# DLR-RM/AugmentedAutoencoder

Hardware: NVIDIA H100
Metric: pose queries/sec (encode+codebook NN) (higher is better)
Workload: dtype f32 via split-fp16 tensor-core products (3x, fp32 accumulate)

## Files before the change

augmentedautoencoder_b200/csrc/tc_common.cuh:

```cuda
#pragma once
#include <cuda.h>
#include <cuda_fp16.h>
#include <cuda_runtime.h>
#include <stdint.h>

namespace aae {
namespace tc {

__device__ __forceinline__ uint32_t smem_u32(const void* p) { return (uint32_t)__cvta_generic_to_shared(p); }

__device__ __forceinline__ bool elect_one() {
  uint32_t pred = 0;
  asm volatile(
      "{\n\t"
      ".reg .pred P1;\n\t"
      "elect.sync _|P1, 0xffffffff;\n\t"
      "selp.b32 %0, 1, 0, P1;\n\t"
      "}\n"
      : "=r"(pred));
  return pred != 0;
}

__device__ __forceinline__ void mbar_init(uint64_t* bar, uint32_t count) {
  asm volatile("mbarrier.init.shared::cta.b64 [%0], %1;" ::"r"(smem_u32(bar)), "r"(count));
}
__device__ __forceinline__ void fence_barrier_init() { asm volatile("fence.mbarrier_init.release.cluster;" ::: "memory"); }
__device__ __forceinline__ void fence_proxy_async_smem() { asm volatile("fence.proxy.async.shared::cta;" ::: "memory"); }

__device__ __forceinline__ void mbar_arrive_expect_tx(uint64_t* bar, uint32_t bytes) {
  asm volatile("mbarrier.arrive.expect_tx.shared::cta.b64 _, [%0], %1;" ::"r"(smem_u32(bar)), "r"(bytes) : "memory");
}
__device__ __forceinline__ void mbar_arrive(uint64_t* bar) {
  asm volatile("mbarrier.arrive.shared::cta.b64 _, [%0];" ::"r"(smem_u32(bar)) : "memory");
}
__device__ __forceinline__ bool mbar_try_wait(uint64_t* bar, uint32_t parity) {
  uint32_t ok;
  asm volatile(
      "{\n\t"
      ".reg .pred P1;\n\t"
      "mbarrier.try_wait.parity.shared::cta.b64 P1, [%1], %2;\n\t"
      "selp.b32 %0, 1, 0, P1;\n\t"
      "}\n"
      : "=r"(ok)
      : "r"(smem_u32(bar)), "r"(parity)
      : "memory");
  return ok != 0;
}
__device__ __forceinline__ void mbar_wait(uint64_t* bar, uint32_t parity) {
  while (!mbar_try_wait(bar, parity)) {
  }
}

__device__ __forceinline__ void prefetch_tmap(const CUtensorMap* m) {
  asm volatile("prefetch.tensormap [%0];" ::"l"(reinterpret_cast<uint64_t>(m)) : "memory");
}
__device__ __forceinline__ void tma_load_2d(void* smem_dst, const CUtensorMap* m, uint64_t* bar, int c0, int c1) {
  asm volatile("cp.async.bulk.tensor.2d.shared::cluster.global.mbarrier::complete_tx::bytes [%0], [%1, {%3, %4}], [%2];" ::"r"(
                   smem_u32(smem_dst)),
               "l"(reinterpret_cast<uint64_t>(m)), "r"(smem_u32(bar)), "r"(c0), "r"(c1)
               : "memory");
}
__device__ __forceinline__ void tma_load_4d(void* smem_dst, const CUtensorMap* m, uint64_t* bar, int c0, int c1, int c2, int c3) {
  asm volatile(
      "cp.async.bulk.tensor.4d.shared::cluster.global.mbarrier::complete_tx::bytes [%0], [%1, {%3, %4, %5, %6}], [%2];" ::"r"(
          smem_u32(smem_dst)),
      "l"(reinterpret_cast<uint64_t>(m)), "r"(smem_u32(bar)), "r"(c0), "r"(c1), "r"(c2), "r"(c3)
      : "memory");
}

__device__ __forceinline__ void bulk_store_1d(void* gmem_dst, const void* smem_src, uint32_t bytes) {
  asm volatile("cp.async.bulk.global.shared::cta.bulk_group [%0], [%1], %2;" ::"l"(gmem_dst), "r"(smem_u32(smem_src)), "r"(bytes) : "memory");
}
__device__ __forceinline__ void bulk_commit_group() { asm volatile("cp.async.bulk.commit_group;" ::: "memory"); }
__device__ __forceinline__ void bulk_wait_read_all() { asm volatile("cp.async.bulk.wait_group.read 0;" ::: "memory"); }
__device__ __forceinline__ void bulk_wait_all() { asm volatile("cp.async.bulk.wait_group 0;" ::: "memory"); }
__device__ __forceinline__ void tma_store_2d(const CUtensorMap* m, const void* smem_src, int c0, int c1) {
  asm volatile("cp.async.bulk.tensor.2d.global.shared::cta.bulk_group [%0, {%2, %3}], [%1];" ::"l"(reinterpret_cast<uint64_t>(m)),
               "r"(smem_u32(smem_src)), "r"(c0), "r"(c1)
               : "memory");
}
__device__ __forceinline__ void tma_store_5d(const CUtensorMap* m, const void* smem_src, int c0, int c1, int c2, int c3, int c4) {
  asm volatile("cp.async.bulk.tensor.5d.global.shared::cta.bulk_group [%0, {%2, %3, %4, %5, %6}], [%1];" ::"l"(reinterpret_cast<uint64_t>(m)),
               "r"(smem_u32(smem_src)), "r"(c0), "r"(c1), "r"(c2), "r"(c3), "r"(c4)
               : "memory");
}

template <int N>
struct Wgmma;
#define AAE_D8(i) "+f"(d[i]), "+f"(d[i + 1]), "+f"(d[i + 2]), "+f"(d[i + 3]), "+f"(d[i + 4]), "+f"(d[i + 5]), "+f"(d[i + 6]), "+f"(d[i + 7])
template <>
struct Wgmma<64> {
  template <int TA, int TB>
  static __device__ __forceinline__ void ss(float (&d)[32], uint64_t da, uint64_t db, uint32_t accumulate) {
    asm volatile(
        "{\n\t.reg .pred p;\n\tsetp.ne.b32 p, %34, 0;\n\t"
        "wgmma.mma_async.sync.aligned.m64n64k16.f32.f16.f16 {%0, %1, %2, %3, %4, %5, %6, %7, %8, %9, %10, %11, %12, %13, %14, %15, %16, %17, %18, %19, %20, %21, %22, %23, %24, %25, %26, %27, %28, %29, %30, %31}, %32, %33, p, 1, 1, %35, %36;\n\t}\n"
        : AAE_D8(0), AAE_D8(8), AAE_D8(16), AAE_D8(24)
        : "l"(da), "l"(db), "r"(accumulate), "n"(TA), "n"(TB));
  }
};

template <>
struct Wgmma<128> {
  template <int TA, int TB>
  static __device__ __forceinline__ void ss(float (&d)[64], uint64_t da, uint64_t db, uint32_t accumulate) {
    asm volatile(
        "{\n\t.reg .pred p;\n\tsetp.ne.b32 p, %66, 0;\n\t"
        "wgmma.mma_async.sync.aligned.m64n128k16.f32.f16.f16 {%0, %1, %2, %3, %4, %5, %6, %7, %8, %9, %10, %11, %12, %13, %14, %15, %16, %17, %18, %19, %20, %21, %22, %23, %24, %25, %26, %27, %28, %29, %30, %31, %32, %33, %34, %35, %36, %37, %38, %39, %40, %41, %42, %43, %44, %45, %46, %47, %48, %49, %50, %51, %52, %53, %54, %55, %56, %57, %58, %59, %60, %61, %62, %63}, %64, %65, p, 1, 1, %67, %68;\n\t}\n"
        : AAE_D8(0), AAE_D8(8), AAE_D8(16), AAE_D8(24), AAE_D8(32), AAE_D8(40), AAE_D8(48), AAE_D8(56)
        : "l"(da), "l"(db), "r"(accumulate), "n"(TA), "n"(TB));
  }
};

__device__ __forceinline__ void wgmma_fence() { asm volatile("wgmma.fence.sync.aligned;" ::: "memory"); }
__device__ __forceinline__ void wgmma_commit() { asm volatile("wgmma.commit_group.sync.aligned;" ::: "memory"); }
template <int N>
__device__ __forceinline__ void wgmma_wait() { asm volatile("wgmma.wait_group.sync.aligned %0;" ::"n"(N) : "memory"); }
template <int R>
__device__ __forceinline__ void wgmma_fence_regs(float (&d)[R]) {
#pragma unroll
  for (int i = 0; i < R; ++i) asm volatile("" : "+f"(d[i])::"memory");
}

template <int N>
__device__ __forceinline__ void setmaxnreg_dec() { asm volatile("setmaxnreg.dec.sync.aligned.u32 %0;" ::"n"(N)); }
template <int N>
__device__ __forceinline__ void setmaxnreg_inc() { asm volatile("setmaxnreg.inc.sync.aligned.u32 %0;" ::"n"(N)); }

__device__ __forceinline__ void cp_async_16(void* smem_dst, const void* gmem_src, bool pred) {
  const int bytes = pred ? 16 : 0;
  asm volatile("cp.async.cg.shared.global [%0], [%1], 16, %2;" ::"r"(smem_u32(smem_dst)), "l"(gmem_src), "r"(bytes) : "memory");
}
__device__ __forceinline__ void cp_async_wait_all() { asm volatile("cp.async.wait_all;" ::: "memory"); }
__device__ __forceinline__ void named_bar_sync(int id, int threads) { asm volatile("bar.sync %0, %1;" ::"r"(id), "r"(threads) : "memory"); }

__device__ __forceinline__ uint64_t make_sw128_kmajor_desc(uint32_t smem_addr) {
  uint64_t d = 0;
  d |= (uint64_t)((smem_addr & 0x3FFFF) >> 4);
  d |= (uint64_t)1 << 16;
  d |= (uint64_t)(1024 >> 4) << 32;
  d |= (uint64_t)1 << 62;
  return d;
}
__device__ __forceinline__ uint64_t make_sw128_mnmajor_desc(uint32_t smem_addr, uint32_t lbo_bytes, uint32_t sbo_bytes) {
  uint64_t d = 0;
  d |= (uint64_t)((smem_addr & 0x3FFFF) >> 4);
  d |= (uint64_t)(lbo_bytes >> 4) << 16;
  d |= (uint64_t)(sbo_bytes >> 4) << 32;
  d |= (uint64_t)1 << 62;
  return d;
}
__device__ __forceinline__ uint64_t desc_advance_k(uint64_t desc, int k_step) { return desc + (uint64_t)((k_step * 32) >> 4); }

__device__ __forceinline__ void split_f16(float x, __half& hi, __half& lo) {
  hi = __float2half_rn(x);
  lo = __float2half_rn(x - __half2float(hi));
}

__device__ __forceinline__ void split_f16x2(float a, float b, uint32_t& hi2, uint32_t& lo2) {
  const float ca = __fmul_rn(a, 8193.0f), cb = __fmul_rn(b, 8193.0f);
  const float ha = __fsub_rn(ca, __fsub_rn(ca, a)), hb = __fsub_rn(cb, __fsub_rn(cb, b));
  const __half2 h = __floats2half2_rn(ha, hb);
  const __half2 l = __floats2half2_rn(__fsub_rn(a, ha), __fsub_rn(b, hb));
  hi2 = *reinterpret_cast<const uint32_t*>(&h);
  lo2 = *reinterpret_cast<const uint32_t*>(&l);
}

}

typedef CUresult (*PFN_tmapEncodeTiled)(CUtensorMap*, CUtensorMapDataType, cuuint32_t, void*, const cuuint64_t*, const cuuint64_t*,
                                        const cuuint32_t*, const cuuint32_t*, CUtensorMapInterleave, CUtensorMapSwizzle,
                                        CUtensorMapL2promotion, CUtensorMapFloatOOBfill);
PFN_tmapEncodeTiled get_tmap_encoder();
int make_tmap_f16(CUtensorMap* out, const void* base, int rank, const uint64_t* dims, const uint64_t* strides_bytes, const uint32_t* box,
                  int swizzle_bytes = 128);

}
```

augmentedautoencoder_b200/csrc/tc_gemm.cu:

```cuda
#include <limits.h>

#include <algorithm>
#include <vector>

#include "tc.cuh"
#include "tc_common.cuh"
#include "tc_plan.cuh"

namespace aae {

using namespace tc;

PFN_tmapEncodeTiled get_tmap_encoder() {
  static PFN_tmapEncodeTiled fn = nullptr;
  if (!fn) {
    void* p = nullptr;
    cudaDriverEntryPointQueryResult q;
    if (cudaGetDriverEntryPoint("cuTensorMapEncodeTiled", &p, cudaEnableDefault, &q) == cudaSuccess && q == cudaDriverEntryPointSuccess)
      fn = reinterpret_cast<PFN_tmapEncodeTiled>(p);
  }
  return fn;
}

int make_tmap_f16(CUtensorMap* out, const void* base, int rank, const uint64_t* dims, const uint64_t* strides_bytes, const uint32_t* box,
                  int swizzle_bytes) {
  PFN_tmapEncodeTiled enc = get_tmap_encoder();
  if (!enc) { set_error("cuTensorMapEncodeTiled is unavailable in this driver"); return AAE_ERR_CUDA; }
  cuuint64_t gdim[5], gstr[4];
  cuuint32_t bx[5], es[5];
  for (int i = 0; i < rank; ++i) { gdim[i] = dims[i]; bx[i] = box[i]; es[i] = 1; }
  for (int i = 0; i + 1 < rank; ++i) gstr[i] = strides_bytes[i];
  CUresult r = enc(out, CU_TENSOR_MAP_DATA_TYPE_FLOAT16, (cuuint32_t)rank, const_cast<void*>(base), gdim, gstr, bx, es,
                   CU_TENSOR_MAP_INTERLEAVE_NONE, swizzle_bytes == 64 ? CU_TENSOR_MAP_SWIZZLE_64B : CU_TENSOR_MAP_SWIZZLE_128B,
                   CU_TENSOR_MAP_L2_PROMOTION_L2_256B,
                   CU_TENSOR_MAP_FLOAT_OOB_FILL_NONE);
  if (r != CUDA_SUCCESS) { set_error("cuTensorMapEncodeTiled failed with CUresult %d (rank %d)", (int)r, rank); return AAE_ERR_CUDA; }
  return AAE_OK;
}

template <int N_TILE, int W_STAGES, int PLANES = 2>
struct TcSmem {
  static constexpr int W_BYTES = N_TILE * TC_KCH * 2;
  static constexpr int W_STAGE_BYTES = PLANES * W_BYTES;
  static constexpr int BODY = TC_A_RING_BYTES + W_STAGES * W_STAGE_BYTES;
  static constexpr int TOTAL = BODY + 1024  + 256 ;
};

struct TcTile {
  int m0, n0, z, u_begin, u_end;
};
template <int N_TILE>
__device__ __forceinline__ TcTile tc_tile(const TcGemmParams& p, const TcTiles& g, int t) {
  TcTile r;
  const int yz = t / g.n;
  const int y = yz % g.m;
  r.z = yz / g.m;
  r.m0 = y * 128;
  r.n0 = (t - yz * g.n) * N_TILE;
  r.u_begin = r.z * p.units_per_split;
  r.u_end = min(p.groups * p.chunks_per_tap, r.u_begin + p.units_per_split);
  return r;
}

template <int N_TILE, int W_STAGES, int PLANES = 2>
__global__ void __launch_bounds__(TC_THREADS, 1)
tc_gemm_kernel(const __grid_constant__ CUtensorMap tm_a_hi, const __grid_constant__ CUtensorMap tm_a_lo,
               const __grid_constant__ CUtensorMap tm_w_hi, const __grid_constant__ CUtensorMap tm_w_lo, const TcGemmParams p,
               const TcTiles tiles) {
  using S = TcSmem<N_TILE, W_STAGES, PLANES>;
  constexpr int R = N_TILE / 2;
  extern __shared__ uint8_t smem_raw[];
  uint8_t* smem = reinterpret_cast<uint8_t*>((reinterpret_cast<uintptr_t>(smem_raw) + 1023) & ~(uintptr_t)1023);
  uint64_t* a_full = reinterpret_cast<uint64_t*>(smem + S::BODY);
  uint64_t* a_empty = a_full + TC_A_SLOTS_MAX;
  uint64_t* w_full = a_empty + TC_A_SLOTS_MAX;
  uint64_t* w_empty = w_full + W_STAGES;
  uint8_t* w_ring = smem + TC_A_RING_BYTES;
  const int a_plane = p.a_rows * TC_KCH * 2, a_slot = PLANES * a_plane;

  const int warp = threadIdx.x >> 5;
  const int lane = threadIdx.x & 31;

  if (threadIdx.x == 0) {
    prefetch_tmap(&tm_a_hi);
    if constexpr (PLANES == 2) prefetch_tmap(&tm_a_lo);
    prefetch_tmap(&tm_w_hi);
    if constexpr (PLANES == 2) prefetch_tmap(&tm_w_lo);
    for (int s = 0; s < p.a_slots; ++s) { mbar_init(&a_full[s], 1); mbar_init(&a_empty[s], 2); }
    for (int s = 0; s < W_STAGES; ++s) { mbar_init(&w_full[s], 1); mbar_init(&w_empty[s], 2); }
    fence_barrier_init();
  }
  __syncthreads();

  if (warp < 4) {
    setmaxnreg_dec<TC_PRODUCER_REGS>();
    if (warp == 0 && lane == 0) {
      const int hw = p.OH * p.OW;
      int ia = 0, iw = 0;
      for (int t = blockIdx.x; t < tiles.count; t += gridDim.x) {
        const TcTile T = tc_tile<N_TILE>(p, tiles, t);
        const int b0 = T.m0 / hw, rem = T.m0 - b0 * hw;
        const int oh0 = rem / p.OW, ow0 = rem - oh0 * p.OW;
        for (int u = T.u_begin; u < T.u_end; ++u, ++ia) {
          const int g = u / p.chunks_per_tap, cc = u - g * p.chunks_per_tap;
          const int sa = ia & (p.a_slots - 1);
          mbar_wait(&a_empty[sa], (ia & p.a_slots) ? 0u : 1u);
          uint8_t* a = smem + sa * a_slot;
          mbar_arrive_expect_tx(&a_full[sa], a_slot);
          const int c0 = p.grp_ch[g] + cc * TC_KCH;
          const int x = ow0 + p.grp_dx[g], y = oh0 + p.grp_dy[g];
          tma_load_4d(a, &tm_a_hi, &a_full[sa], c0, x, y, b0);
          if constexpr (PLANES == 2) tma_load_4d(a + a_plane, &tm_a_lo, &a_full[sa], c0, x, y, b0);
          const int first = p.grp_first[g], ntaps = p.grp_ntaps[g];
          for (int k = 0; k < ntaps; ++k, ++iw) {
            const int sw = iw % W_STAGES;
            mbar_wait(&w_empty[sw], ((uint32_t)(iw / W_STAGES) & 1u) ^ 1u);
            uint8_t* w = w_ring + sw * S::W_STAGE_BYTES;
            mbar_arrive_expect_tx(&w_full[sw], S::W_STAGE_BYTES);
            const int kcol = (p.grp_tap[first + k] * p.chunks_per_tap + cc) * TC_KCH;
            tma_load_2d(w, &tm_w_hi, &w_full[sw], kcol, T.n0);
            if constexpr (PLANES == 2) tma_load_2d(w + S::W_BYTES, &tm_w_lo, &w_full[sw], kcol, T.n0);
          }
        }
      }
    }
  } else {
    setmaxnreg_inc<TC_CONSUMER_REGS>();
    const int wg = (warp - 4) >> 2;
    const bool releases = (warp & 3) == 0 && lane == 0;
    constexpr int H = R / 8;
    float acc[R], crs[R], v[R];
#pragma unroll
    for (int j = 0; j < R; ++j) { acc[j] = 0.f; crs[j] = 0.f; v[j] = 0.f; }
    int pt = 0, half = 2;
    auto epilogue_half = [&](int h) {
      const TcTile P = tc_tile<N_TILE>(p, tiles, pt);
      if (h == 0) tc_epilogue_frag<PLANES, 0, H>(p, v, P.m0 + wg * 64, P.n0, P.z, warp, lane);
      else tc_epilogue_frag<PLANES, H, 2 * H>(p, v, P.m0 + wg * 64, P.n0, P.z, warp, lane);
    };
    int ia = 0, iw = 0;
    for (int t = blockIdx.x; t < tiles.count; t += gridDim.x) {
      const TcTile T = tc_tile<N_TILE>(p, tiles, t);
      for (int u = T.u_begin; u < T.u_end; ++u, ++ia) {
        const int g = u / p.chunks_per_tap;
        const int sa = ia & (p.a_slots - 1);
        mbar_wait(&a_full[sa], (ia & p.a_slots) ? 1u : 0u);
        const int first = p.grp_first[g], ntaps = p.grp_ntaps[g];
        for (int k = 0; k < ntaps; ++k, ++iw) {
          const int sw = iw % W_STAGES;
          mbar_wait(&w_full[sw], (uint32_t)(iw / W_STAGES) & 1u);
          const uint32_t a_tap = smem_u32(smem + sa * a_slot) + (uint32_t)((wg * p.a_wg_rows + p.grp_row[first + k]) * TC_KCH * 2);
          const uint32_t st = smem_u32(w_ring + sw * S::W_STAGE_BYTES);
          const uint64_t a_hi = make_sw128_kmajor_desc(a_tap);
          const uint64_t a_lo = make_sw128_kmajor_desc(a_tap + (uint32_t)a_plane);
          const uint64_t w_hi = make_sw128_kmajor_desc(st);
          const uint64_t w_lo = make_sw128_kmajor_desc(st + S::W_BYTES);
          const bool accumulate = u > T.u_begin || k > 0;
          wgmma_fence_regs(acc);
          if constexpr (PLANES == 2) wgmma_fence_regs(crs);
          wgmma_fence();
#pragma unroll
          for (int kk = 0; kk < TC_KCH / 16; ++kk) {
            const uint32_t scale_d = (accumulate || kk > 0) ? 1u : 0u;
            Wgmma<N_TILE>::template ss<0, 0>(acc, desc_advance_k(a_hi, kk), desc_advance_k(w_hi, kk), scale_d);
            if constexpr (PLANES == 2) {
              Wgmma<N_TILE>::template ss<0, 0>(crs, desc_advance_k(a_lo, kk), desc_advance_k(w_hi, kk), scale_d);
              Wgmma<N_TILE>::template ss<0, 0>(crs, desc_advance_k(a_hi, kk), desc_advance_k(w_lo, kk), 1u);
            }
          }
          wgmma_commit();
          if (half < 2) epilogue_half(half++);
          wgmma_wait<1>();
          wgmma_fence_regs(acc);
          if constexpr (PLANES == 2) wgmma_fence_regs(crs);
          if (accumulate && releases) {
            mbar_arrive(&w_empty[(iw - 1) % W_STAGES]);
            if (k == 0) mbar_arrive(&a_empty[(ia - 1) & (p.a_slots - 1)]);
          }
        }
      }
      wgmma_wait<0>();
      wgmma_fence_regs(acc);
      if constexpr (PLANES == 2) wgmma_fence_regs(crs);
      const bool has_work = T.u_end > T.u_begin;
      if (has_work && releases) {
        mbar_arrive(&w_empty[(iw - 1) % W_STAGES]);
        mbar_arrive(&a_empty[(ia - 1) & (p.a_slots - 1)]);
      }
      while (half < 2) epilogue_half(half++);
      tc_epilogue_values<PLANES>(p, acc, crs, has_work, v);
      pt = t; half = 0;
    }
    while (half < 2) epilogue_half(half++);
  }
}

namespace {

template <int PLANES>
__global__ void pack_weights_kernel(const float* __restrict__ w, int taps, int cin, int cout, float scale, __half* __restrict__ hi,
                                    __half* __restrict__ lo, unsigned* __restrict__ range_flag, unsigned range_bit) {
  __shared__ float tile[32][33];
  const int tap = blockIdx.z;
  const int ci0 = blockIdx.y * 32, co0 = blockIdx.x * 32;
  for (int i = threadIdx.y; i < 32; i += 8) {
    const int ci = ci0 + i, co = co0 + threadIdx.x;
    tile[i][threadIdx.x] = (ci < cin && co < cout) ? w[((long long)tap * cin + ci) * cout + co] : 0.f;
  }
  __syncthreads();
  for (int i = threadIdx.y; i < 32; i += 8) {
    const int co = co0 + i, ci = ci0 + threadIdx.x;
    if (co < cout && ci < cin)
      tc_store_f16<PLANES>(tile[threadIdx.x][i] * scale, hi, lo, (long long)co * taps * cin + (long long)tap * cin + ci, range_flag, range_bit);
  }
}

template <int PLANES>
__global__ void unpack_act_kernel(const __half* __restrict__ hi, const __half* __restrict__ lo, int B, int H, int W, int C, int s2d,
                                  float inv_scale, float* __restrict__ out) {
  const long long total = (long long)B * H * W * C;
  for (long long i = (long long)blockIdx.x * blockDim.x + threadIdx.x; i < total; i += (long long)gridDim.x * blockDim.x) {
    const int c = (int)(i % C);
    long long r = i / C;
    const int w = (int)(r % W); r /= W;
    const int h = (int)(r % H);
    const int b = (int)(r / H);
    long long src = i;
    if (s2d) src = ((long long)(b * (H >> 1) + (h >> 1)) * (W >> 1) + (w >> 1)) * (4LL * C) + (((h & 1) << 1) | (w & 1)) * C + c;
    out[i] = tc_load_f16<PLANES>(hi, lo, src) * inv_scale;
  }
}

}

namespace {

template <int PLANES>
__global__ void __launch_bounds__(256) splitk_forward_finish_kernel(const float* __restrict__ partials, int splits, const TcGemmParams p) {
  const long long groups = (long long)p.M * (p.N >> 3);
  for (long long gi = (long long)blockIdx.x * blockDim.x + threadIdx.x; gi < groups; gi += (long long)gridDim.x * blockDim.x) {
    const int m = (int)(gi / (p.N >> 3)), n = (int)(gi - (long long)m * (p.N >> 3)) << 3;
    float f[8] = {0.f, 0.f, 0.f, 0.f, 0.f, 0.f, 0.f, 0.f};
    const float* src = partials + (long long)m * p.N + n;
    for (int sp = 0; sp < splits; ++sp, src += (long long)p.M * p.N) {
      const float4 a = *reinterpret_cast<const float4*>(src), b = *reinterpret_cast<const float4*>(src + 4);
      f[0] += a.x; f[1] += a.y; f[2] += a.z; f[3] += a.w; f[4] += b.x; f[5] += b.y; f[6] += b.z; f[7] += b.w;
    }
    float amax = 0.f;
#pragma unroll
    for (int j = 0; j < 8; ++j) {
      float v = f[j] + (p.bias ? __ldg(p.bias + n + j) : 0.f);
      if (p.relu == 1) v = fmaxf(v, 0.f);
      amax = fmaxf(amax, fabsf(v));
      f[j] = v * p.out_scale;
    }
    if (p.range_flag != nullptr && !(amax * p.out_scale < TC_F16_OVERFLOW)) atomicOr(p.range_flag, p.range_bit);
    tc_store_f16<PLANES>(f, 1.f, p.out_hi, p.out_lo, tc_decode_row(p, m).row_off + n);
  }
}

int dev_alloc(void** p, size_t bytes) { return tc_dev_alloc(p, bytes); }

int scratch_grow(void** p, size_t bytes, cudaStream_t s) {
  cudaFree(*p);
  *p = nullptr;
  cudaError_t e = cudaMalloc(p, bytes);
  if (e != cudaSuccess) { *p = nullptr; set_error("cudaMalloc(%zu) failed: %s", bytes, cudaGetErrorString(e)); return AAE_ERR_OOM; }
  AAE_CUDA_OK(cudaMemsetAsync(*p, 0, bytes, s));
  return AAE_OK;
}

bool pow2(int v) { return v > 0 && (v & (v - 1)) == 0; }

}

int tc_dev_alloc(void** p, size_t bytes) {
  cudaError_t e = cudaMalloc(p, bytes);
  if (e != cudaSuccess) { *p = nullptr; set_error("cudaMalloc(%zu) failed: %s", bytes, cudaGetErrorString(e)); return AAE_ERR_OOM; }
  cudaMemset(*p, 0, bytes);
  return AAE_OK;
}

int TcPlanes::alloc(size_t n, int planes) {
  AAE_TRY(tc_dev_alloc((void**)&hi, n * sizeof(__half)));
  return planes == 2 ? tc_dev_alloc((void**)&lo, n * sizeof(__half)) : AAE_OK;
}

void TcPlanes::release() {
  cudaFree(hi);
  cudaFree(lo);
  hi = lo = nullptr;
}

int TcPlanes::encode(TcMaps& m, int rank, const uint64_t* dims, const uint64_t* strides_bytes, const uint32_t* box, int swizzle_bytes) const {
  AAE_TRY(make_tmap_f16(&m.hi, hi, rank, dims, strides_bytes, box, swizzle_bytes));
  if (lo == nullptr) {
    m.lo = m.hi;
    return AAE_OK;
  }
  return make_tmap_f16(&m.lo, lo, rank, dims, strides_bytes, box, swizzle_bytes);
}

constexpr int TC_W_STAGES_SPLIT = 3, TC_W_STAGES_FP16 = 6;
static_assert(TcSmem<TC_N_TILE, TC_W_STAGES_FP16, 1>::TOTAL == TcSmem<TC_N_TILE, TC_W_STAGES_SPLIT>::TOTAL, "same footprint");
static_assert(TcSmem<TC_N_TILE, TC_W_STAGES_SPLIT>::TOTAL <= 227 * 1024, "tc_gemm_kernel: shared memory over the sm_90 limit");

int tc_plan_groups(TcLayer& T, int planes, const uint64_t* dims, const uint64_t* strides_bytes) {
  TcGemmParams& g = T.gp;
  AAE_REQUIRE(g.taps >= 1 && g.taps <= 32, "tc plan: %d taps (at most 32)", g.taps);
  AAE_REQUIRE(T.BW * T.BH * T.BB == 128, "tc plan: box %d x %d x %d is not one 128-row tile", T.BW, T.BH, T.BB);
  const int halo_rows = (T.BH + 2) * T.BW * T.BB;
  bool halo = g.taps > 1 && T.BW % 8 == 0 && (T.BB == 1 || (T.BB == 2 && T.BH * T.BW == 64)) &&
              2 * planes * halo_rows * TC_KCH * 2 <= TC_A_RING_BYTES && T.BH + 2 <= 256;
  for (int t = 0; t < g.taps; ++t) halo = halo && g.tap_di[t] >= -1 && g.tap_di[t] <= 1;
  g.groups = 0;
  for (int t = 0; t < g.taps; ++t) {
    int grp = -1;
    for (int q = 0; halo && q < g.groups; ++q)
      if (g.grp_ch[q] == g.tap_ch[t] && g.grp_dx[q] == g.tap_dj[t]) grp = q;
    if (grp < 0) {
      grp = g.groups++;
      g.grp_ch[grp] = g.tap_ch[t];
      g.grp_dx[grp] = g.tap_dj[t];
      g.grp_dy[grp] = (int8_t)(halo ? -1 : g.tap_di[t]);
      g.grp_ntaps[grp] = 0;
    }
    g.grp_ntaps[grp]++;
  }
  int n = 0;
  for (int q = 0; q < g.groups; ++q) {
    g.grp_first[q] = (int8_t)n;
    for (int t = 0; t < g.taps; ++t) {
      if (halo ? (g.grp_ch[q] != g.tap_ch[t] || g.grp_dx[q] != g.tap_dj[t]) : t != q) continue;
      g.grp_tap[n] = (int8_t)t;
      g.grp_row[n] = (int16_t)(halo ? (g.tap_di[t] + 1) * T.BW : 0);
      ++n;
    }
  }
  AAE_REQUIRE(n == g.taps, "tc plan: tap groups cover %d of %d taps", n, g.taps);
  g.a_rows = halo ? halo_rows : 128;
  g.a_wg_rows = halo && T.BB == 2 ? (T.BH + 2) * T.BW : 64;
  const int slot_bytes = planes * g.a_rows * TC_KCH * 2;
  g.a_slots = 1;
  while (2 * g.a_slots <= TC_A_SLOTS_MAX && 2 * g.a_slots * slot_bytes <= TC_A_RING_BYTES) g.a_slots *= 2;
  AAE_REQUIRE(g.a_slots >= 2, "tc plan: an A slot of %d bytes leaves fewer than two in the ring", slot_bytes);
  AAE_REQUIRE(g.a_rows % 8 == 0 && g.a_wg_rows % 8 == 0, "tc plan: A box rows %d / warpgroup offset %d off the 8-row atom", g.a_rows, g.a_wg_rows);
  for (int i = 0; i < n; ++i) AAE_REQUIRE(g.grp_row[i] % 8 == 0 && g.grp_row[i] + g.a_wg_rows + 64 <= g.a_rows, "tc plan: tap row %d outside the A box", g.grp_row[i]);
  g.units_per_split = g.groups * g.chunks_per_tap;
  if (!halo) return AAE_OK;
  const uint32_t box[4] = {(uint32_t)TC_KCH, (uint32_t)T.BW, (uint32_t)(T.BH + 2), (uint32_t)T.BB};
  return T.in.encode(T.tm_halo, 4, dims, strides_bytes, box);
}

int tc_launch_layer(const TcLayer& T, dim3 tiles, cudaStream_t s, int planes) {
  const long long count = (long long)tiles.x * tiles.y * tiles.z;
  AAE_REQUIRE(count <= INT_MAX, "tc_gemm: %lld tiles exceed the kernel's int tile index", count);
  AAE_REQUIRE(T.gp.a_slots >= 2 && T.gp.a_slots <= TC_A_SLOTS_MAX && (T.gp.a_slots & (T.gp.a_slots - 1)) == 0 &&
              T.gp.a_slots * planes * T.gp.a_rows * TC_KCH * 2 <= TC_A_RING_BYTES, "tc_gemm: layer without a tap-group plan");
  int device = 0, sms = 0;
  AAE_CUDA_OK(cudaGetDevice(&device));
  AAE_CUDA_OK(cudaDeviceGetAttribute(&sms, cudaDevAttrMultiProcessorCount, device));
  const TcTiles g{(int)tiles.y, (int)tiles.x, (int)count};
  const unsigned ctas = (unsigned)std::min<long long>(count, sms);
  const TcMaps& a = T.gp.a_rows == 128 ? T.tm_a : T.tm_halo;
  return with_planes(planes, [&](auto P) {
    constexpr int W_STAGES = P == 1 ? TC_W_STAGES_FP16 : TC_W_STAGES_SPLIT;
    using S = TcSmem<TC_N_TILE, W_STAGES, P>;
    auto kern = tc_gemm_kernel<TC_N_TILE, W_STAGES, P>;
    AAE_CUDA_OK(cudaFuncSetAttribute(kern, cudaFuncAttributeMaxDynamicSharedMemorySize, S::TOTAL));
    kern<<<ctas, TC_THREADS, S::TOTAL, s>>>(a.hi, a.lo, T.tm_w.hi, T.tm_w.lo, T.gp, g);
    AAE_LAUNCH_OK();
    return AAE_OK;
  });
}

int tc_encoder_create(int device, const aae_net_cfg* cfg, TcEncoder** out) {
  *out = nullptr;
  const int L = cfg->num_layers;
  AAE_REQUIRE(aae_device_supported(device), "AAE_PREC_TC_SPLIT needs a compute-capability 9.0 device (wgmma/TMA)");
  if (L < 2) {
    set_error("AAE_PREC_TC_SPLIT: at least two conv layers expected (this network has %d)", L);
    return AAE_ERR_UNSUPPORTED;
  }
  const int planes = tc_planes(cfg->precision);
  if (planes == 1 && !tc_conv1_supported(cfg)) {
    set_error("AAE_PREC_TC_FP16: the first layer needs the tensor-core conv1 (128 x 128 x 3 crops, 128 filters, k = 5, stride 2)");
    return AAE_ERR_UNSUPPORTED;
  }
  TcEncoder* h = new TcEncoder();
  h->device = device;
  h->cfg = *cfg;
  h->planes = planes;
  int ih = (cfg->in_h + cfg->strides[0] - 1) / cfg->strides[0], iw = (cfg->in_w + cfg->strides[0] - 1) / cfg->strides[0], ic = cfg->filters[0];
  const int B = cfg->max_batch;
  int st = AAE_OK;
  for (int l = 1; l <= L && st == AAE_OK; ++l) {
    TcLayer T;
    memset(&T.gp, 0, sizeof(T.gp));
    const bool dense = (l == L);
    if (!dense) {
      if (cfg->strides[l] != 2 || cfg->kernel_size != 5 || (ih & 1) || (iw & 1) || ic % 64 != 0 || cfg->filters[l] % 32 != 0) {
        set_error("AAE_PREC_TC_SPLIT: layer %d unsupported (needs k=5, stride 2, even dims, Cin %% 64 == 0, Cout %% 32 == 0)", l);
        st = AAE_ERR_UNSUPPORTED;
        break;
      }
      T.in_h = ih; T.in_w = iw; T.in_c = ic;
      T.out_h = ih / 2; T.out_w = iw / 2; T.out_c = cfg->filters[l];
      T.taps = 25;
      if (!pow2(T.out_w) || !pow2(T.out_h) || T.out_w > 128) { set_error("AAE_PREC_TC_SPLIT: output dims must be powers of two <= 128"); st = AAE_ERR_UNSUPPORTED; break; }
      T.BW = T.out_w;
      T.BH = std::min(T.out_h, 128 / T.BW);
      T.BB = 128 / (T.BW * T.BH);
    } else {
      T.in_h = T.in_w = 1; T.in_c = ih * iw * ic;
      T.out_h = T.out_w = 1; T.out_c = cfg->latent;
      T.taps = 1; T.BW = 1; T.BH = 1; T.BB = 128;
      h->flat = T.in_c;
      if (T.in_c % 64 != 0 || T.out_c % 32 != 0) { set_error("AAE_PREC_TC_SPLIT: dense layer needs flat %% 64 == 0 and latent %% 32 == 0"); st = AAE_ERR_UNSUPPORTED; break; }
    }
    const int B_pad = (int)ceil_div(B, T.BB) * T.BB;
    const int w_rows = (int)ceil_div(T.out_c, TC_N_TILE) * TC_N_TILE;
    if ((st = T.in.alloc((size_t)B_pad * T.in_h * T.in_w * T.in_c, planes)) != AAE_OK) break;
    if ((st = T.w.alloc((size_t)w_rows * T.taps * T.in_c, planes)) != AAE_OK) break;
    uint64_t a_dims[4], a_strides[3];
    if (!dense) {
      const uint64_t C4 = 4ull * T.in_c, W2 = T.in_w / 2, H2 = T.in_h / 2;
      const uint64_t dims[4] = {C4, W2, H2, (uint64_t)B_pad};
      const uint64_t strides[3] = {C4 * 2, W2 * C4 * 2, H2 * W2 * C4 * 2};
      memcpy(a_dims, dims, sizeof(dims)); memcpy(a_strides, strides, sizeof(strides));
    } else {
      const uint64_t dims[4] = {(uint64_t)T.in_c, 1, 1, (uint64_t)B_pad};
      const uint64_t strides[3] = {(uint64_t)T.in_c * 2, (uint64_t)T.in_c * 2, (uint64_t)T.in_c * 2};
      memcpy(a_dims, dims, sizeof(dims)); memcpy(a_strides, strides, sizeof(strides));
    }
    {
      const uint32_t box[4] = {(uint32_t)TC_KCH, (uint32_t)T.BW, (uint32_t)T.BH, (uint32_t)T.BB};
      if ((st = T.in.encode(T.tm_a, 4, a_dims, a_strides, box)) != AAE_OK) break;
    }
    {
      const uint64_t K = (uint64_t)T.taps * T.in_c;
      const uint64_t dims[2] = {K, (uint64_t)w_rows};
      const uint64_t strides[1] = {K * 2};
      const uint32_t box[2] = {(uint32_t)TC_KCH, (uint32_t)TC_N_TILE};
      if ((st = T.w.encode(T.tm_w, 2, dims, strides, box)) != AAE_OK) break;
    }
    TcGemmParams& g = T.gp;
    g.N = T.out_c; g.OH = T.out_h; g.OW = T.out_w; g.BW = T.BW; g.BH = T.BH;
    g.taps = T.taps; g.chunks_per_tap = T.in_c / TC_KCH;
    for (int t = 0; t < T.taps; ++t) {
      if (dense) { g.tap_di[t] = 0; g.tap_dj[t] = 0; g.tap_ch[t] = 0; continue; }
      const int kh = t / 5, kw = t % 5;
      g.tap_di[t] = (int8_t)((kh + 1) / 2 - 1);
      g.tap_dj[t] = (int8_t)((kw + 1) / 2 - 1);
      g.tap_ch[t] = ((((kh + 1) & 1) << 1) | ((kw + 1) & 1)) * T.in_c;
    }
    if ((st = tc_plan_groups(T, planes, a_dims, a_strides)) != AAE_OK) break;
    g.unscale = 1.f / (ACT_SCALE * W_SCALE);
    g.out_scale = ACT_SCALE;
    g.relu = dense ? 0 : 1;
    h->layers.push_back(T);
    if (!dense) { ih = T.out_h; iw = T.out_w; ic = T.out_c; }
  }
  if (st == AAE_OK) {
    for (size_t i = 0; i + 1 < h->layers.size(); ++i) {
      TcGemmParams& g = h->layers[i].gp;
      g.out_hi = h->layers[i + 1].in.hi;
      g.out_lo = h->layers[i + 1].in.lo;
      g.out_mode = (i + 2 == h->layers.size()) ? OUT_PLAIN_SPLIT : OUT_S2D_SPLIT;
    }
    TcLayer& D = h->layers.back();
    const int total = D.gp.groups * D.gp.chunks_per_tap;
    h->dense_splits = std::min(total, 66);
    D.gp.units_per_split = (total + h->dense_splits - 1) / h->dense_splits;
    h->dense_splits = (total + D.gp.units_per_split - 1) / D.gp.units_per_split;
    D.gp.out_mode = OUT_F32;
    st = dev_alloc((void**)&h->partials, (size_t)h->dense_splits * (B + 128) * cfg->latent * sizeof(float));
    D.gp.out_f32 = h->partials;
  }
  if (st == AAE_OK) st = dev_alloc((void**)&h->range_flag, sizeof(unsigned));
  if (st == AAE_OK)
    for (size_t i = 0; i + 1 < h->layers.size(); ++i) {
      h->layers[i].gp.range_flag = h->range_flag;
      h->layers[i].gp.range_bit = 1u << (i + 1);
    }
  if (st == AAE_OK && tc_conv1_supported(cfg)) st = tc_conv1_create(device, cfg, &h->conv1);
  if (st != AAE_OK) { tc_encoder_destroy(h); return st; }
  *out = h;
  return AAE_OK;
}

void tc_encoder_destroy(TcEncoder* h) {
  if (!h) return;
  for (auto& T : h->layers) { T.in.release(); T.w.release(); }
  cudaFree(h->partials);
  cudaFree(h->fwd_partials);
  cudaFree(h->dbg);
  if (h->owns_range_flag) cudaFree(h->range_flag);
  tc_conv1_destroy(h->conv1);
  delete h;
}

int tc_encoder_pack_weights(TcEncoder* h, int layer, const float* w_dev, cudaStream_t s) {
  if (layer == 0) {
    if (h->conv1) return tc_conv1_pack(h->conv1, w_dev, h->cfg.kernel_size * h->cfg.kernel_size * h->cfg.in_c, W_SCALE, h->range_flag, 1u << 16, s);
    return AAE_OK;
  }
  AAE_REQUIRE(layer >= 1 && layer <= (int)h->layers.size(), "tc pack: layer %d out of range", layer);
  TcLayer& T = h->layers[layer - 1];
  dim3 grid((unsigned)ceil_div(T.out_c, 32), (unsigned)ceil_div(T.in_c, 32), (unsigned)T.taps), block(32, 8);
  with_planes(h->planes, [&](auto P) {
    pack_weights_kernel<P><<<grid, block, 0, s>>>(w_dev, T.taps, T.in_c, T.out_c, W_SCALE, T.w.hi, T.w.lo, h->range_flag, 1u << (16 + layer));
  });
  AAE_LAUNCH_OK();
  return AAE_OK;
}

unsigned* tc_encoder_range_flag(TcEncoder* h) { return h->range_flag; }
unsigned* tc_decoder_range_flag(TcDecoder* h) { return h->range_flag; }

void tc_encoder_share_range_flag(TcEncoder* h, unsigned* flag) {
  if (h->owns_range_flag) cudaFree(h->range_flag);
  h->range_flag = flag;
  h->owns_range_flag = false;
  for (size_t i = 0; i + 1 < h->layers.size(); ++i) h->layers[i].gp.range_flag = flag;
}

void tc_decoder_share_range_flag(TcDecoder* h, unsigned* flag) {
  if (h->owns_range_flag) cudaFree(h->range_flag);
  h->range_flag = flag;
  h->owns_range_flag = false;
  for (size_t i = 0; i + 1 < h->layers.size(); ++i) h->layers[i].gp.range_flag = flag;
}

int tc_encoder_forward(TcEncoder* h, const void* crops, int src_u8, int B, const float* w0, const float* b0, const float* dense_b,
                       float* z_out, StageTimer* timer, cudaStream_t s) {
  const aae_net_cfg& cfg = h->cfg;
  timer->reset();
  timer->mark(s);
  if (h->conv1) {
    AAE_TRY(tc_conv1_forward(h->conv1, &cfg, crops, src_u8, B, b0, ACT_SCALE, W_SCALE, h->layers[0].in.hi, h->layers[0].in.lo, h->range_flag, s));
  } else {
    IGemmParams p;
    memset(&p, 0, sizeof(p));
    p.src = crops; p.src_u8 = src_u8;
    p.B = B; p.SH = cfg.in_h; p.SW = cfg.in_w; p.SC = cfg.in_c;
    p.PH = h->layers[0].in_h; p.PW = h->layers[0].in_w;
    p.KH = p.KW = cfg.kernel_size; p.stride = cfg.strides[0];
    const int tot_h = std::max((p.PH - 1) * p.stride + p.KH - cfg.in_h, 0), tot_w = std::max((p.PW - 1) * p.stride + p.KW - cfg.in_w, 0);
    p.pad_t = tot_h / 2; p.pad_l = tot_w / 2;
    p.Bm = w0; p.N = cfg.filters[0]; p.bias = b0; p.act = ACT_RELU;
    p.M = B * p.PH * p.PW; p.K = p.KH * p.KW * p.SC;
    p.k_per_split = (int)ceil_div(p.K, 16) * 16;
    p.split_hi = h->layers[0].in.hi; p.split_lo = h->layers[0].in.lo; p.split_scale = ACT_SCALE; p.split_s2d = 1;
    p.range_flag = h->range_flag; p.range_bit = 1u;
    AAE_TRY(launch_igemm(p, GATHER_FWD, s));
  }
  timer->mark(s);
  for (size_t i = 0; i < h->layers.size(); ++i) {
    TcLayer& T = h->layers[i];
    const bool dense = (i + 1 == h->layers.size());
    T.gp.M = dense ? B : B * T.out_h * T.out_w;
    dim3 grid((unsigned)ceil_div(T.gp.M, 128), (unsigned)ceil_div(T.out_c, TC_N_TILE), dense ? (unsigned)h->dense_splits : 1u);
    int splits = 1;
    if (!dense && T.gp.out_mode != OUT_F32) {
      const int tiles = (int)(grid.x * grid.y), total_iters = T.gp.taps * T.gp.chunks_per_tap;
      if (tiles * 2 <= 132) {
        splits = std::min(132 / tiles, std::max(1, total_iters / 24));
        const size_t per_split = (size_t)T.gp.M * T.gp.N;
        if (per_split * (size_t)splits > h->fwd_partial_floats) {
          const size_t want = std::min<size_t>(per_split * (size_t)splits, (size_t)32 << 20);
          if (want > h->fwd_partial_floats) {
            h->fwd_partial_floats = 0;
            AAE_TRY(scratch_grow((void**)&h->fwd_partials, want * sizeof(float), s));
            h->fwd_partial_floats = want;
          }
          splits = (int)std::min<size_t>((size_t)splits, h->fwd_partial_floats / per_split);
        }
        splits = std::max(splits, 1);
      }
    }
    if (splits > 1) {
      TcLayer S = T;
      const int total_units = T.gp.groups * T.gp.chunks_per_tap;
      S.gp.units_per_split = (int)ceil_div(total_units, splits);
      splits = (int)ceil_div(total_units, S.gp.units_per_split);
      S.gp.out_mode = OUT_F32;
      S.gp.out_f32 = h->fwd_partials;
      grid.z = (unsigned)splits;
      AAE_TRY(tc_launch_layer(S, grid, s, h->planes));
      const long long groups = (long long)T.gp.M * (T.gp.N >> 3);
      const unsigned fin_grid = (unsigned)std::min<long long>(132 * 8, ceil_div(groups, 256));
      with_planes(h->planes, [&](auto P) { splitk_forward_finish_kernel<P><<<fin_grid, 256, 0, s>>>(h->fwd_partials, splits, T.gp); });
      AAE_LAUNCH_OK();
    } else {
      AAE_TRY(tc_launch_layer(T, grid, s, h->planes));
    }
    if (dense) AAE_TRY(launch_splitk_reduce(h->partials, h->dense_splits, (int64_t)B * cfg.latent, cfg.latent, dense_b, ACT_NONE, z_out, s));
    timer->mark(s);
  }
  return AAE_OK;
}

int tc_encoder_set_bias(TcEncoder* h, int layer, const float* bias_dev) {
  if (layer >= 1 && layer < (int)h->layers.size()) h->layers[layer - 1].gp.bias = bias_dev;
  return AAE_OK;
}

int tc_encoder_activation(TcEncoder* h, int layer, int B, const float** ptr, int64_t* count, cudaStream_t s) {
  AAE_REQUIRE(layer >= 0 && layer < (int)h->layers.size(), "tc activation: layer %d out of range", layer);
  const TcLayer& T = h->layers[layer];
  const bool plain = (layer + 1 == (int)h->layers.size());
  int H, W, C;
  if (plain) { const TcLayer& P = h->layers[layer - 1]; H = P.out_h; W = P.out_w; C = P.out_c; }
  else { H = T.in_h; W = T.in_w; C = T.in_c; }
  const size_t n = (size_t)B * H * W * C;
  if (h->dbg_floats < n) {
    h->dbg_floats = 0;
    AAE_TRY(scratch_grow((void**)&h->dbg, n * sizeof(float), s));
    h->dbg_floats = n;
  }
  with_planes(h->planes, [&](auto P) {
    unpack_act_kernel<P><<<1024, 256, 0, s>>>(T.in.hi, T.in.lo, B, H, W, C, plain ? 0 : 1, 1.f / ACT_SCALE, h->dbg);
  });
  AAE_LAUNCH_OK();
  AAE_CUDA_OK(cudaStreamSynchronize(s));
  *ptr = h->dbg;
  *count = (int64_t)n;
  return AAE_OK;
}


namespace {

template <int PLANES>
__global__ void split_scale_kernel(const float* __restrict__ x, long long n, float scale, __half* __restrict__ hi, __half* __restrict__ lo,
                                   unsigned* __restrict__ range_flag, unsigned range_bit) {
  for (long long i = (long long)blockIdx.x * blockDim.x + threadIdx.x; i < n; i += (long long)gridDim.x * blockDim.x)
    tc_store_f16<PLANES>(x[i] * scale, hi, lo, i, range_flag, range_bit);
}

template <int PLANES>
__global__ void pack_out_sep_kernel(const float* __restrict__ wm, int cin, int n4, int rows, float scale, __half* __restrict__ hi,
                                    __half* __restrict__ lo, unsigned* __restrict__ range_flag, unsigned range_bit) {
  const int total = rows * cin;
  for (int i = blockIdx.x * blockDim.x + threadIdx.x; i < total; i += gridDim.x * blockDim.x) {
    const int ci = i % cin, n = i / cin;
    const int tap = n / n4, m = n - tap * n4;
    tc_store_f16<PLANES>(tap < 9 ? wm[((long long)tap * cin + ci) * n4 + m] * scale : 0.f, hi, lo, i, range_flag, range_bit);
  }
}

__global__ void outlayer_gather_kernel(const float* __restrict__ P, int ldp, const float* __restrict__ bias, const float* __restrict__ mask_bias,
                                       int B, int h, int w, int c, int cm, float* __restrict__ x, float* __restrict__ mask) {
  const int ct = c + cm, n4 = 4 * ct;
  const long long total = (long long)B * h * w * n4;
  for (long long t = (long long)blockIdx.x * blockDim.x + threadIdx.x; t < total; t += (long long)gridDim.x * blockDim.x) {
    const int m = (int)(t % n4);
    long long r = t / n4;
    const int j = (int)(r % w); r /= w;
    const int i = (int)(r % h);
    const long long b = r / h;
    const int cls = m / ct, co = m - cls * ct;
    const float* bp = co < c ? bias : mask_bias;
    float s = bp ? __ldg(bp + (co < c ? co : 0)) : 0.f;
#pragma unroll
    for (int ty = 0; ty < 3; ++ty) {
      const int ii = i + ty - 1;
      if (ii < 0 || ii >= h) continue;
#pragma unroll
      for (int tx = 0; tx < 3; ++tx) {
        const int jj = j + tx - 1;
        if (jj < 0 || jj >= w) continue;
        s += P[((b * h + ii) * w + jj) * ldp + (ty * 3 + tx) * n4 + m];
      }
    }
    const long long px = (b * 2 * h + 2 * i + (cls >> 1)) * (2LL * w) + 2 * j + (cls & 1);
    if (co < c) x[px * c + co] = 1.f / (1.f + expf(-s));
    else if (mask) mask[px] = 1.f / (1.f + expf(-s));
  }
}

__global__ void tile_bias_kernel(const float* __restrict__ b, int cout, float* __restrict__ out) {
  const int i = blockIdx.x * blockDim.x + threadIdx.x;
  if (i < 4 * cout) out[i] = b[i % cout];
}

}

int tc_layer_setup_plain(TcLayer& T, int B, int planes) {
  const int B_pad = (int)ceil_div(B, T.BB) * T.BB;
  const uint64_t K = (uint64_t)T.taps * T.in_c;
  const int rows = (int)ceil_div(T.gp.N, TC_N_TILE) * TC_N_TILE;
  AAE_TRY(T.in.alloc((size_t)B_pad * T.in_h * T.in_w * T.in_c, planes));
  AAE_TRY(T.w.alloc((size_t)rows * K, planes));
  {
    const uint64_t dims[4] = {(uint64_t)T.in_c, (uint64_t)T.in_w, (uint64_t)T.in_h, (uint64_t)B_pad};
    const uint64_t strides[3] = {(uint64_t)T.in_c * 2, (uint64_t)T.in_w * T.in_c * 2, (uint64_t)T.in_h * T.in_w * T.in_c * 2};
    const uint32_t box[4] = {(uint32_t)TC_KCH, (uint32_t)T.BW, (uint32_t)T.BH, (uint32_t)T.BB};
    AAE_TRY(T.in.encode(T.tm_a, 4, dims, strides, box));
    AAE_TRY(tc_plan_groups(T, planes, dims, strides));
  }
  const uint64_t dims[2] = {K, (uint64_t)rows};
  const uint64_t strides[1] = {K * 2};
  const uint32_t box[2] = {(uint32_t)TC_KCH, (uint32_t)TC_N_TILE};
  return T.w.encode(T.tm_w, 2, dims, strides, box);
}

int tc_decoder_create(int device, const aae_net_cfg* cfg, bool mask_head, TcDecoder** out) {
  *out = nullptr;
  AAE_REQUIRE(aae_device_supported(device), "AAE_PREC_TC_SPLIT needs a compute-capability 9.0 device (wgmma/TMA)");
  const int L = cfg->num_layers;
  if (cfg->kernel_size != 5 || cfg->in_h != cfg->in_w) {
    set_error("AAE_PREC_TC_SPLIT decoder: kernel 5 and square crops required (kernel %d, %d x %d crops)", cfg->kernel_size, cfg->in_h, cfg->in_w);
    return AAE_ERR_UNSUPPORTED;
  }
  TcDecoder* h = new TcDecoder();
  h->device = device;
  h->cfg = *cfg;
  h->planes = tc_planes(cfg->precision);
  const int B = cfg->max_batch;
  int h0 = cfg->in_h;
  for (int i = 0; i < L; ++i) h0 /= 2;
  std::vector<int> nf(L);
  for (int i = 0; i < L; ++i) nf[i] = cfg->filters[L - 1 - i];
  int st = AAE_OK;
  for (int l = 0; l <= L && st == AAE_OK; ++l) {
    TcLayer T;
    memset(&T.gp, 0, sizeof(T.gp));
    TcGemmParams& g = T.gp;
    if (l == 0) {
      T.in_h = T.in_w = 1; T.in_c = cfg->latent; T.out_h = T.out_w = 1; T.out_c = h0 * h0 * nf[0];
      T.taps = 1; T.BW = 1; T.BH = 1; T.BB = 128;
      g.N = T.out_c; g.OH = g.OW = 1; g.relu = 1; g.out_mode = OUT_PLAIN_SPLIT;
      if (cfg->latent % 64 != 0 || T.out_c % 128 != 0) { set_error("tc decoder: latent %% 64 and dense width %% 128 required"); st = AAE_ERR_UNSUPPORTED; break; }
    } else {
      const int hh = h0 << (l - 1);
      T.in_h = T.in_w = hh; T.in_c = nf[l - 1];
      const int cout = l < L ? nf[l] : cfg->in_c + (mask_head ? 1 : 0);
      T.out_h = T.out_w = 2 * hh; T.out_c = cout;
      T.taps = 9;
      if (hh > 128 || (hh & (hh - 1)) || T.in_c % 64 != 0 || (l < L && cout % 64 != 0)) {
        set_error("tc decoder: layer %d unsupported (power-of-two size <= 128, Cin %% 64, Cout %% 64)", l); st = AAE_ERR_UNSUPPORTED; break;
      }
      T.BW = hh; T.BH = std::min(hh, 128 / T.BW); T.BB = 128 / (T.BW * T.BH);
      g.OH = g.OW = hh;
      if (l < L) { g.N = 4 * cout; g.relu = 1; g.out_mode = OUT_D2S_SPLIT; }
      else {
        if (cfg->in_c > 3) {
          set_error("tc decoder: %d output channels, the tensor-core output layer takes at most 3 (AAE_PREC_FP32_SIMT takes any count)", cfg->in_c);
          st = AAE_ERR_UNSUPPORTED; break;
        }
        T.taps = 1; g.N = (int)ceil_div(36 * cout, 128) * 128; g.relu = 0; g.out_mode = OUT_F32;
        h->out_x = cfg->in_c;
        st = dev_alloc((void**)&h->out_p, (size_t)ceil_div((int64_t)B * hh * hh, 128) * 128 * g.N * sizeof(float));
        if (st == AAE_OK && mask_head) st = dev_alloc((void**)&h->cat_tmp, (size_t)25 * T.in_c * cout * sizeof(float));
        if (st != AAE_OK) break;
      }
    }
    g.BW = T.BW; g.BH = T.BH; g.taps = T.taps; g.chunks_per_tap = T.in_c / TC_KCH;
    for (int t = 0; t < T.taps; ++t) {
      g.tap_di[t] = (int8_t)(T.taps == 1 ? 0 : t / 3 - 1);
      g.tap_dj[t] = (int8_t)(T.taps == 1 ? 0 : t % 3 - 1);
      g.tap_ch[t] = 0;
    }
    g.unscale = 1.f / (ACT_SCALE * W_SCALE);
    g.out_scale = ACT_SCALE;
    if ((st = tc_layer_setup_plain(T, B, h->planes)) != AAE_OK) { h->layers.push_back(T); break; }
    h->layers.push_back(T);
    float* bz = nullptr;
    if (l > 0 && l < L) st = dev_alloc((void**)&bz, (size_t)g.N * sizeof(float));
    h->bias_dev.push_back(bz);
    h->wm_floats = std::max(h->wm_floats, (size_t)9 * T.in_c * 4 * T.out_c);
  }
  if (st == AAE_OK) st = dev_alloc((void**)&h->wm_tmp, h->wm_floats * sizeof(float));
  if (st == AAE_OK) st = dev_alloc((void**)&h->range_flag, sizeof(unsigned));
  if (st == AAE_OK) {
    for (size_t i = 0; i + 1 < h->layers.size(); ++i) {
      h->layers[i].gp.out_hi = h->layers[i + 1].in.hi;
      h->layers[i].gp.out_lo = h->layers[i + 1].in.lo;
      h->layers[i].gp.range_flag = h->range_flag;
      h->layers[i].gp.range_bit = 1u << i;
    }
  }
  if (st != AAE_OK) { tc_decoder_destroy(h); return st; }
  *out = h;
  return AAE_OK;
}

void tc_decoder_destroy(TcDecoder* h) {
  if (!h) return;
  for (auto& T : h->layers) { T.in.release(); T.w.release(); }
  for (auto b : h->bias_dev) cudaFree(b);
  cudaFree(h->wm_tmp);
  cudaFree(h->out_p);
  cudaFree(h->cat_tmp);
  if (h->owns_range_flag) cudaFree(h->range_flag);
  delete h;
}

int tc_decoder_pack_weights(TcDecoder* h, int layer, const float* w_dev, const float* b_dev, cudaStream_t s) {
  AAE_REQUIRE(layer >= 0 && layer < (int)h->layers.size(), "tc decoder pack: layer %d out of range", layer);
  TcLayer& T = h->layers[layer];
  dim3 block(32, 8);
  if (layer == 0) {
    if (w_dev) {
      dim3 grid((unsigned)ceil_div(T.out_c, 32), (unsigned)ceil_div(T.in_c, 32), 1);
      with_planes(h->planes, [&](auto P) {
        pack_weights_kernel<P><<<grid, block, 0, s>>>(w_dev, 1, T.in_c, T.out_c, W_SCALE, T.w.hi, T.w.lo, h->range_flag, 1u << 16);
      });
      AAE_LAUNCH_OK();
    }
    if (b_dev) T.gp.bias = b_dev;
    return AAE_OK;
  }
  const bool out_layer = layer + 1 == (int)h->layers.size();
  if (w_dev) {
    if (out_layer && h->cat_tmp) {
      AAE_REQUIRE(h->mask_w != nullptr, "tc decoder: the mask head's weights are not set");
      AAE_TRY(launch_copy_channels(w_dev, h->out_x, 0, h->cat_tmp, T.out_c, 0, h->out_x, 25LL * T.in_c, s));
      AAE_TRY(launch_copy_channels(h->mask_w, 1, 0, h->cat_tmp, T.out_c, h->out_x, 1, 25LL * T.in_c, s));
      w_dev = h->cat_tmp;
    }
    AAE_TRY(launch_merge_subpixel_weights(w_dev, T.in_c, T.out_c, h->wm_tmp, s));
    const unsigned bit = 1u << (16 + layer);
    dim3 grid((unsigned)ceil_div(4 * T.out_c, 32), (unsigned)ceil_div(T.in_c, 32), 9);
    with_planes(h->planes, [&](auto P) {
      if (out_layer) pack_out_sep_kernel<P><<<64, 256, 0, s>>>(h->wm_tmp, T.in_c, 4 * T.out_c, T.gp.N, W_SCALE, T.w.hi, T.w.lo, h->range_flag, bit);
      else pack_weights_kernel<P><<<grid, block, 0, s>>>(h->wm_tmp, 9, T.in_c, 4 * T.out_c, W_SCALE, T.w.hi, T.w.lo, h->range_flag, bit);
    });
    AAE_LAUNCH_OK();
  }
  if (out_layer) {
    if (b_dev) h->out_bias = b_dev;
    return AAE_OK;
  }
  if (b_dev) {
    tile_bias_kernel<<<(unsigned)ceil_div(T.gp.N, 128), 128, 0, s>>>(b_dev, T.out_c, h->bias_dev[layer]);
    AAE_LAUNCH_OK();
    T.gp.bias = h->bias_dev[layer];
  }
  return AAE_OK;
}

const float* tc_decoder_merged_weights(const TcDecoder* h) { return h->wm_tmp; }

void tc_decoder_set_mask_head(TcDecoder* h, const float* w_dev, const float* b_dev) {
  h->mask_w = w_dev;
  h->mask_b = b_dev;
}

int tc_decoder_forward(TcDecoder* h, const float* z_dev, int B, float* x_out, float* mask_out, cudaStream_t s) {
  TcLayer& D = h->layers[0];
  const unsigned grid = (unsigned)std::min<int64_t>(1024, ceil_div((int64_t)B * D.in_c, 256));
  with_planes(h->planes, [&](auto P) {
    split_scale_kernel<P><<<grid, 256, 0, s>>>(z_dev, (long long)B * D.in_c, ACT_SCALE, D.in.hi, D.in.lo, h->range_flag, 1u << 15);
  });
  AAE_LAUNCH_OK();
  for (size_t i = 0; i < h->layers.size(); ++i) {
    TcLayer& T = h->layers[i];
    T.gp.M = i == 0 ? B : B * T.in_h * T.in_w;
    const bool last = i + 1 == h->layers.size();
    if (last) T.gp.out_f32 = h->out_p;
    dim3 grid((unsigned)ceil_div(T.gp.M, 128), (unsigned)ceil_div(T.gp.N, TC_N_TILE), 1u);
    AAE_TRY(tc_launch_layer(T, grid, s, h->planes));
    if (last) {
      const long long total = (long long)T.gp.M * 4 * T.out_c;
      outlayer_gather_kernel<<<(unsigned)std::min<long long>(132 * 16, ceil_div(total, 256)), 256, 0, s>>>(
          h->out_p, T.gp.N, h->out_bias, h->mask_b, B, T.in_h, T.in_w, h->out_x, T.out_c - h->out_x, x_out, mask_out);
      AAE_LAUNCH_OK();
    }
  }
  return AAE_OK;
}

}
```

Before: 50750.

## Merge hi and lo weight-plane wgmmas into one double-width N instruction

The lo and hi weight planes now sit next to each other in shared memory, so a_hi times [w_lo|w_hi] is issued as a single m64n(2N) wgmma whose output covers the cross and main accumulators held in one contiguous register array. This replaces two of the three split-fp16 wgmma issues per k-step with one wider instruction, cutting issue overhead and A-operand rereads. It changes the order of accumulation into the cross term and relies on the combined register array staying within the consumer register budget, and an N=256 fragment raises register pressure.

```diff
diff --git a/augmentedautoencoder_b200/csrc/tc_common.cuh b/augmentedautoencoder_b200/csrc/tc_common.cuh
--- a/augmentedautoencoder_b200/csrc/tc_common.cuh
+++ b/augmentedautoencoder_b200/csrc/tc_common.cuh
@@ -112,6 +112,25 @@
   }
 };
 
+template <>
+struct Wgmma<256> {
+  template <int TA, int TB>
+  static __device__ __forceinline__ void ss(float (&d)[128], uint64_t da, uint64_t db, uint32_t accumulate) {
+    asm volatile(
+        "{\n\t.reg .pred p;\n\tsetp.ne.b32 p, %130, 0;\n\t"
+        "wgmma.mma_async.sync.aligned.m64n256k16.f32.f16.f16 {%0, %1, %2, %3, %4, %5, %6, %7, %8, %9, %10, %11, %12, %13, %14, %15, %16, %17, %18, %19, %20, %21, %22, %23, %24, %25, %26, %27, %28, %29, %30, %31, %32, %33, %34, %35, %36, %37, %38, %39, %40, %41, %42, %43, %44, %45, %46, %47, %48, %49, %50, %51, %52, %53, %54, %55, %56, %57, %58, %59, %60, %61, %62, %63, %64, %65, %66, %67, %68, %69, %70, %71, %72, %73, %74, %75, %76, %77, %78, %79, %80, %81, %82, %83, %84, %85, %86, %87, %88, %89, %90, %91, %92, %93, %94, %95, %96, %97, %98, %99, %100, %101, %102, %103, %104, %105, %106, %107, %108, %109, %110, %111, %112, %113, %114, %115, %116, %117, %118, %119, %120, %121, %122, %123, %124, %125, %126, %127}, %128, %129, p, 1, 1, %131, %132;\n\t}\n"
+        : AAE_D8(0), AAE_D8(8), AAE_D8(16), AAE_D8(24), AAE_D8(32), AAE_D8(40), AAE_D8(48), AAE_D8(56), AAE_D8(64), AAE_D8(72), AAE_D8(80),
+          AAE_D8(88), AAE_D8(96), AAE_D8(104), AAE_D8(112), AAE_D8(120)
+        : "l"(da), "l"(db), "r"(accumulate), "n"(TA), "n"(TB));
+  }
+};
+
+template <int OFF, int N, int M>
+__device__ __forceinline__ float (&frag_part(float (&d)[M]))[N] {
+  static_assert(OFF >= 0 && OFF + N <= M, "frag_part: outside the fragment");
+  return *reinterpret_cast<float(*)[N]>(d + OFF);
+}
+
 __device__ __forceinline__ void wgmma_fence() { asm volatile("wgmma.fence.sync.aligned;" ::: "memory"); }
 __device__ __forceinline__ void wgmma_commit() { asm volatile("wgmma.commit_group.sync.aligned;" ::: "memory"); }
 template <int N>
diff --git a/augmentedautoencoder_b200/csrc/tc_gemm.cu b/augmentedautoencoder_b200/csrc/tc_gemm.cu
--- a/augmentedautoencoder_b200/csrc/tc_gemm.cu
+++ b/augmentedautoencoder_b200/csrc/tc_gemm.cu
@@ -41,6 +41,7 @@
 template <int N_TILE, int W_STAGES, int PLANES = 2>
 struct TcSmem {
   static constexpr int W_BYTES = N_TILE * TC_KCH * 2;
+  static constexpr int W_HI_OFF = (PLANES - 1) * W_BYTES;
   static constexpr int W_STAGE_BYTES = PLANES * W_BYTES;
   static constexpr int BODY = TC_A_RING_BYTES + W_STAGES * W_STAGE_BYTES;
   static constexpr int TOTAL = BODY + 1024  + 256 ;
@@ -118,8 +119,8 @@
             uint8_t* w = w_ring + sw * S::W_STAGE_BYTES;
             mbar_arrive_expect_tx(&w_full[sw], S::W_STAGE_BYTES);
             const int kcol = (p.grp_tap[first + k] * p.chunks_per_tap + cc) * TC_KCH;
-            tma_load_2d(w, &tm_w_hi, &w_full[sw], kcol, T.n0);
-            if constexpr (PLANES == 2) tma_load_2d(w + S::W_BYTES, &tm_w_lo, &w_full[sw], kcol, T.n0);
+            tma_load_2d(w + S::W_HI_OFF, &tm_w_hi, &w_full[sw], kcol, T.n0);
+            if constexpr (PLANES == 2) tma_load_2d(w, &tm_w_lo, &w_full[sw], kcol, T.n0);
           }
         }
       }
@@ -129,9 +130,13 @@
     const int wg = (warp - 4) >> 2;
     const bool releases = (warp & 3) == 0 && lane == 0;
     constexpr int H = R / 8;
-    float acc[R], crs[R], v[R];
+    float F[2 * R], v[R];
+    float(&acc)[R] = frag_part<(PLANES - 1) * R, R>(F);
+    float(&crs)[R] = frag_part<(2 - PLANES) * R, R>(F);
 #pragma unroll
-    for (int j = 0; j < R; ++j) { acc[j] = 0.f; crs[j] = 0.f; v[j] = 0.f; }
+    for (int j = 0; j < 2 * R; ++j) F[j] = 0.f;
+#pragma unroll
+    for (int j = 0; j < R; ++j) v[j] = 0.f;
     int pt = 0, half = 2;
     auto epilogue_half = [&](int h) {
       const TcTile P = tc_tile<N_TILE>(p, tiles, pt);
@@ -153,26 +158,27 @@
           const uint32_t st = smem_u32(w_ring + sw * S::W_STAGE_BYTES);
           const uint64_t a_hi = make_sw128_kmajor_desc(a_tap);
           const uint64_t a_lo = make_sw128_kmajor_desc(a_tap + (uint32_t)a_plane);
-          const uint64_t w_hi = make_sw128_kmajor_desc(st);
-          const uint64_t w_lo = make_sw128_kmajor_desc(st + S::W_BYTES);
+          const uint64_t w_hi = make_sw128_kmajor_desc(st + S::W_HI_OFF);
+          const uint64_t w_lo_hi = make_sw128_kmajor_desc(st);
           const bool accumulate = u > T.u_begin || k > 0;
-          wgmma_fence_regs(acc);
-          if constexpr (PLANES == 2) wgmma_fence_regs(crs);
+          if constexpr (PLANES == 2) wgmma_fence_regs(F);
+          else wgmma_fence_regs(acc);
           wgmma_fence();
 #pragma unroll
           for (int kk = 0; kk < TC_KCH / 16; ++kk) {
             const uint32_t scale_d = (accumulate || kk > 0) ? 1u : 0u;
-            Wgmma<N_TILE>::template ss<0, 0>(acc, desc_advance_k(a_hi, kk), desc_advance_k(w_hi, kk), scale_d);
             if constexpr (PLANES == 2) {
-              Wgmma<N_TILE>::template ss<0, 0>(crs, desc_advance_k(a_lo, kk), desc_advance_k(w_hi, kk), scale_d);
-              Wgmma<N_TILE>::template ss<0, 0>(crs, desc_advance_k(a_hi, kk), desc_advance_k(w_lo, kk), 1u);
+              Wgmma<2 * N_TILE>::template ss<0, 0>(F, desc_advance_k(a_hi, kk), desc_advance_k(w_lo_hi, kk), scale_d);
+              Wgmma<N_TILE>::template ss<0, 0>(crs, desc_advance_k(a_lo, kk), desc_advance_k(w_hi, kk), 1u);
+            } else {
+              Wgmma<N_TILE>::template ss<0, 0>(acc, desc_advance_k(a_hi, kk), desc_advance_k(w_hi, kk), scale_d);
             }
           }
           wgmma_commit();
           if (half < 2) epilogue_half(half++);
           wgmma_wait<1>();
-          wgmma_fence_regs(acc);
-          if constexpr (PLANES == 2) wgmma_fence_regs(crs);
+          if constexpr (PLANES == 2) wgmma_fence_regs(F);
+          else wgmma_fence_regs(acc);
           if (accumulate && releases) {
             mbar_arrive(&w_empty[(iw - 1) % W_STAGES]);
             if (k == 0) mbar_arrive(&a_empty[(ia - 1) & (p.a_slots - 1)]);
@@ -180,8 +186,8 @@
         }
       }
       wgmma_wait<0>();
-      wgmma_fence_regs(acc);
-      if constexpr (PLANES == 2) wgmma_fence_regs(crs);
+      if constexpr (PLANES == 2) wgmma_fence_regs(F);
+      else wgmma_fence_regs(acc);
       const bool has_work = T.u_end > T.u_begin;
       if (has_work && releases) {
         mbar_arrive(&w_empty[(iw - 1) % W_STAGES]);
```

Result: no change. 50910 (median of 6 runs) (+0.3%).
